# KirillHit/snn_for_object_detection

Measured on AMD Instinct MI355X. Metric: event-frames/sec (BxT) SODa-3M GEN1 304x240 fwd+bwd, higher is better.
Workload: dtype f32 (16-bit split products)

## Files before the change

include/snn_hip.h:

```cpp
#ifndef SNN_HIP_H
#define SNN_HIP_H

#include <stddef.h>
#include <stdint.h>

#ifdef __cplusplus
extern "C" {
#endif

#define SNN_ABI_VERSION 20

enum {
    SNN_NEURON_NONE = 0,
    SNN_NEURON_LIF = 1,
    SNN_NEURON_LI = 2,
    SNN_NEURON_LI_TANH = 3,
    SNN_NEURON_SLI = 4,
    SNN_NEURON_SYNAPSE = 5
};

enum { SNN_PREC_FP32 = 0, SNN_PREC_BF16X3 = 1, SNN_PREC_BF16X6 = 3, SNN_PREC_FP16X3 = 4, SNN_PREC_BF16X1 = 5,
       SNN_PREC_BF16S = 6 };

enum { SNN_SCAN_WIDE_ADDRESSING = 1,
// ... 66 lines not shown
                     int64_t N, int H, int W, int Cin, int Ho, int Wo, int Cout,
                     int KH, int KW, int stride, int pad, const float* addend, int64_t ld_addend,
                     const float* addend2, int64_t ld_addend2, int precision, void* stream);
int snn_conv2d_wgrad(const float* x, int64_t ldx, const float* dy, int64_t lddy, float* dw,
                     int64_t N, int H, int W, int Cin, int Ho, int Wo, int Cout,
                     int KH, int KW, int stride, int pad, int accumulate,
                     float* workspace, int splitk, int precision, void* stream);
int snn_conv2d_wgrad_splitk(int64_t N, int H, int W, int Cin, int Ho, int Wo, int Cout, int KH, int KW,
                            int stride, int pad, int precision);
int snn_conv2d_wgrad_kernel(int64_t N, int H, int W, int Cin, int Ho, int Wo, int Cout, int KH, int KW, int stride, int pad,
                            int precision);
int snn_conv2d_gather_plan(int mode, int64_t N, int H, int W, int Cin, int Ho, int Wo, int Cout, int KH, int KW, int stride,
                           int pad, int64_t ld_in, int64_t ld_out, int align_bits, int has_split_image, int has_addend,
                           int has_addend2, int frames_per_step, int precision, int phase, int* out);
int snn_conv2d_wgrad_plan(int64_t N, int H, int W, int Cin, int Ho, int Wo, int Cout, int KH, int KW, int stride, int pad,
                          int64_t ldx, int64_t lddy, int align_bits, int precision, int spikes, int num_cu, int* out);
int snn_conv1x1_spikes_supported(int64_t N, int H, int W, int Cin, int Cout, int64_t ld, int fwd_precision,
                                 int bwd_precision);
int snn_conv1x1_spikes_fwd(const float* vdec, int64_t ld, float v_th, const float* w, float* y, int64_t ldy, int64_t N, int H,
                           int W, int Cin, int Cout, void* stream);
int snn_conv1x1_spikes_wgrad(const float* vdec, int64_t ld, float v_th, const float* dy, int64_t lddy, float* dw, int64_t N,
                             int H, int W, int Cin, int Cout, int accumulate, float* workspace, int splitk, void* stream);

int snn_conv2d_spikes_supported(int64_t N, int H, int W, int Cin, int Ho, int Wo, int Cout, int KH, int KW, int stride,
                                int pad, int64_t ld, int fwd_precision, int bwd_precision);
int snn_conv2d_spikes_fwd(const float* vdec, int64_t ld, float v_th, const float* w, float* y, int64_t ldy, int64_t N, int H,
                          int W, int Cin, int Ho, int Wo, int Cout, int KH, int KW, int stride, int pad, double* bn_partial,
                          int frames_per_step, int* bn_layout, void* stream);
int snn_conv2d_spikes_wgrad(const float* vdec, int64_t ld, float v_th, const float* dy, int64_t lddy, float* dw, int64_t N,
                            int H, int W, int Cin, int Ho, int Wo, int Cout, int KH, int KW, int stride, int pad,
                            int accumulate, float* workspace, int splitk, void* stream);
int snn_conv3x3_halo_spikes(const float* vdec, int64_t ld, float v_th, const void* w_image, float* y, int64_t ldy, int64_t N,
                            int H, int W, int Cin, int Cout, double* bn_partial, int frames_per_step, int* bn_layout,
                            void* stream);

size_t snn_bn_stats_partial_size(int T, int64_t M, int C);
int snn_bn_stats(const float* y, int64_t ldy, int T, int64_t M, int C, double* partial, void* stream);
int snn_bn_stats_finalize(const double* partial, int chunks, int rows_per_chunk, int T, int64_t M, int C,
                          const float* gamma, const float* bias, float eps, float momentum,
                          float* running_mean, float* running_var, int use_running,
                          float* mean, float* invstd, float* alpha, float* beta, void* stream);

int snn_bn_stats_reduce(const double* partial, int chunks, int rows_per_chunk, int T, int64_t M, int C, double* sums,
                        void* stream);
int snn_bn_stats_from_sums(const double* sums, int T, int64_t M_total, int C,
                           const float* gamma, const float* bias, float eps, float momentum,
// ... 161 lines not shown
```

snn_for_object_detection_amd/_build.py:

```python

import hashlib
import json
import os
import shutil
import subprocess
import sys
from concurrent.futures import ThreadPoolExecutor

HERE = os.path.dirname(os.path.abspath(__file__))
CSRC = os.path.join(HERE, "csrc")
INCLUDE = os.path.join(os.path.dirname(HERE), "include")
SCRATCH = os.path.join(os.path.dirname(HERE), "build")
LIB_NAME = "libsnn_hip.so"
LIB_PATH = os.path.join(HERE, LIB_NAME)
STAMP_PATH = LIB_PATH + ".buildstamp"
SOURCES = ("elementwise.hip", "neuron.hip", "conv.hip", "wgrad_halo.hip", "conv_halo.hip", "detect.hip",
           "targets.hip", "metrics.hip")
HEADERS = (os.path.join(CSRC, "snn_common.h"), os.path.join(INCLUDE, "snn_hip.h"))
ARCH = "gfx950"
FLAGS = ["-O3", f"--offload-arch={ARCH}", "-fPIC", "-ffp-contract=off", "-std=c++17", "-Wall",
         "-Wno-unused-function", f"-I{INCLUDE}"]


def _hipcc() -> str:
    for cand in (os.environ.get("HIPCC"), shutil.which("hipcc"), "/opt/rocm/bin/hipcc"):
        if cand and os.path.exists(cand):
            return cand
    raise RuntimeError("hipcc not found: the HIP extension cannot be built")


def _sha(*chunks: bytes) -> str:
    h = hashlib.sha256()
    for c in chunks:
        h.update(c)
    return h.hexdigest()


def source_fingerprint() -> str:
    h = hashlib.sha256()
# ... 128 lines not shown
```

snn_for_object_detection_amd/_hip.py:

```python

import ctypes
import os
from ctypes import POINTER, Structure, c_char_p, c_double, c_float, c_int, c_int32, c_int64, c_size_t, c_void_p

_HERE = os.path.dirname(os.path.abspath(__file__))
LIB_PATH = os.environ.get("SNN_HIP_LIB") or os.path.join(_HERE, "libsnn_hip.so")

NEURON_NONE, NEURON_LIF, NEURON_LI, NEURON_LI_TANH, NEURON_SLI, NEURON_SYNAPSE = 0, 1, 2, 3, 4, 5
POOL_AVG, POOL_MAX, POOL_SUM = 0, 1, 2
ACT_RELU, ACT_SILU, ACT_TANH = 0, 1, 2
ABI_VERSION = 20
PREC_FP32, PREC_BF16X3, PREC_BF16X6, PREC_FP16X3, PREC_BF16X1, PREC_BF16S = 0, 1, 3, 4, 5, 6
SCAN_WIDE_ADDRESSING, SCAN_LAST_STEP_ONLY, SCAN_BF16_STORAGE, SCAN_SPIKES_FROM_VDEC, SCAN_SUMS_FROM_STATE = 1, 2, 4, 8, 16
SCAN_STATE_LOOKBACK = 32
SURR_SUPER, SURR_TRIANGLE, SURR_SIGMOID, SURR_ATAN = 0, 1, 2, 3


class NeuronParams(Structure):
    _fields_ = [("c_mem", c_float), ("c_syn", c_float), ("v_leak", c_float), ("v_th", c_float),
                ("v_reset", c_float), ("alpha", c_float), ("v_st", c_float), ("tau_sec", c_float),
                ("tau_dis", c_float), ("dt", c_float), ("sigma", c_float),
                ("surrogate", c_int), ("reset_detached", c_int)]


# ... 20 lines not shown
                                    _P, _I, _P]),
    "snn_conv3x3_s2_dgrad_supported": (c_int, [_L, _I, _I, _I, _I, _I, _I]),
    "snn_conv3x3_s2_dgrad_plan": (c_int, [_L, _I, _I, _I, _I, _I, _I, _P]),
    "snn_conv3x3_halo_plan": (c_int, [_L, _I, _I, _I, _I, _I, _P]),
    "snn_conv2d_wgrad_halo_plan": (c_int, [_L, _I, _I, _I, _I, _I, _I, _I, _I, _P]),
    "snn_conv_first_plan": (c_int, [_L, _I, _I, _I, _I, _I, _I, _I, _I, _I, _I, _P]),
    "snn_conv3x3_s2_dgrad": (c_int, [_P, _L, _P, _P, _L, _L, _I, _I, _I, _I, _I, _I, _P, _L, _P, _L, _I, _P]),
    "snn_conv3x3_halo_supported": (c_int, [_L, _I, _I, _I, _I]),
    "snn_conv3x3_halo_bn_chunks": (c_int64, [_I, _I, _I]),
    "snn_weight_frag_image_bytes": (c_size_t, [_I, _I]),
    "snn_weight_frag_image_batched": (c_int, [_P, _P, _P, _I, _I, _I, _I, _P]),
    "snn_conv3x3_halo": (c_int, [_P, _L, _P, _P, _L, _L, _I, _I, _I, _I, _P, _L, _P, _L, _P, _I, _P, _I, _P]),
    "snn_conv2d_dgrad": (c_int, [_P, _L, _P, _P, _P, _L, _L, _I, _I, _I, _I, _I, _I, _I, _I, _I, _I, _P, _L, _P, _L,
                                 _I, _P]),
    "snn_conv2d_wgrad": (c_int, [_P, _L, _P, _L, _P, _L, _I, _I, _I, _I, _I, _I, _I, _I, _I, _I, _I, _P, _I, _I,
                                 _P]),
    "snn_conv2d_wgrad_splitk": (c_int, [_L, _I, _I, _I, _I, _I, _I, _I, _I, _I, _I, _I]),
    "snn_conv2d_wgrad_kernel": (c_int, [_L, _I, _I, _I, _I, _I, _I, _I, _I, _I, _I, _I]),
    "snn_conv2d_gather_plan": (c_int, [_I, _L, _I, _I, _I, _I, _I, _I, _I, _I, _I, _I, _L, _L, _I, _I, _I, _I, _I, _I, _I, _P]),
    "snn_conv2d_wgrad_plan": (c_int, [_L, _I, _I, _I, _I, _I, _I, _I, _I, _I, _I, _L, _L, _I, _I, _I, _I, _P]),
    "snn_conv1x1_spikes_supported": (c_int, [_L, _I, _I, _I, _I, _L, _I, _I]),
    "snn_conv1x1_spikes_fwd": (c_int, [_P, _L, _F, _P, _P, _L, _L, _I, _I, _I, _I, _P]),
    "snn_conv1x1_spikes_wgrad": (c_int, [_P, _L, _F, _P, _L, _P, _L, _I, _I, _I, _I, _I, _P, _I, _P]),
    "snn_conv2d_spikes_supported": (c_int, [_L, _I, _I, _I, _I, _I, _I, _I, _I, _I, _I, _L, _I, _I]),
    "snn_conv2d_spikes_fwd": (c_int, [_P, _L, _F, _P, _P, _L, _L, _I, _I, _I, _I, _I, _I, _I, _I, _I, _I, _P, _I, _P, _P]),
    "snn_conv2d_spikes_wgrad": (c_int, [_P, _L, _F, _P, _L, _P, _L, _I, _I, _I, _I, _I, _I, _I, _I, _I, _I, _I, _P, _I, _P]),
    "snn_conv3x3_halo_spikes": (c_int, [_P, _L, _F, _P, _P, _L, _L, _I, _I, _I, _I, _P, _I, _P, _P]),
    "snn_bn_stats_partial_size": (c_size_t, [_I, _L, _I]),
    "snn_bn_stats": (c_int, [_P, _L, _I, _L, _I, _P, _P]),
    "snn_bn_stats_finalize": (c_int, [_P, _I, _I, _I, _L, _I, _P, _P, _F, _F, _P, _P, _I, _P, _P, _P, _P, _P]),
    "snn_bn_stats_reduce": (c_int, [_P, _I, _I, _I, _L, _I, _P, _P]),
    "snn_bn_stats_from_sums": (c_int, [_P, _I, _L, _I, _P, _P, _F, _F, _P, _P, _P, _P, _P, _P, _P, _P]),
    "snn_bn_bwd_reduce": (c_int, [_P, _I, _L, _I, _P, _P]),
    "snn_bn_bwd_coef": (c_int, [_P, _P, _P, _I, _L, _I, _P, _P, _P, _P, _P, _P, _P, _P, _I, _P]),
    "snn_affine_neuron_fwd": (c_int, [_I, _P, _L, _P, _P, _P, _P, _P, _L, _P, _L, _P, _P, _P, _I, _L, _I,
                                      POINTER(NeuronParams), _I, _P]),
    "snn_lif_ckpt_interval": (c_int, []),
    "snn_lif_fwd_ckpt": (c_int, [_P, _L, _P, _P, _P, _P, _P, _L, _P, _L, _P, _P, _P, _I, _L, _I,
                                 POINTER(NeuronParams), _P]),
    "snn_lif_bwd_ckpt": (c_int, [_P, _L, _P, _P, _L, _P, _P, _P, _P, _I, _P, _P, _P, _P, _I, _L, _I,
                                 POINTER(NeuronParams), _P]),
    "snn_affine_neuron_bwd_sums_size": (c_size_t, [_I, _L, _I]),
    "snn_affine_neuron_bwd": (c_int, [_I, _P, _L, _P, _P, _L, _P, _P, _P, _P, _I, _P, _P, _P, _P, _I, _L, _I,
                                      POINTER(NeuronParams), _I, _P]),
    "snn_bn_bwd_finalize": (c_int, [_P, _I, _L, _I, _P, _P, _P, _P, _P, _P, _P, _P, _I, _P]),
    "snn_bn_bwd_finalize_from_state": (c_int, [_P, _I, _L, _I, _P, _P, _P, _P, _P, _P, _L, _P, _P, _P, _P, _P, _I, _P]),
# ... 91 lines not shown
```

snn_for_object_detection_amd/csrc/conv.hip:

```cpp
#include <stdlib.h>
#include <type_traits>
#include "snn_common.h"

#if defined(SNN_STAMP) || defined(SNN_CLOCK)
__device__ unsigned long long g_stamps[2048 * 8];
__device__ unsigned long long g_stamps2[2048 * 4];
extern "C" int snn_debug_stamps(unsigned long long* out, int n) {
    return (int)hipMemcpyFromSymbol(out, HIP_SYMBOL(g_stamps), sizeof(unsigned long long) * n);
}
extern "C" int snn_debug_stamps2(unsigned long long* out, int n) {
    return (int)hipMemcpyFromSymbol(out, HIP_SYMBOL(g_stamps2), sizeof(unsigned long long) * n);
}
#endif
#ifdef SNN_STAMP
#define STAMP(i) do { unsigned long long t_ = __builtin_readcyclecounter(); st_acc[i] += t_ - st_last; st_last = t_; } while (0)
#else
#define STAMP(i) do {} while (0)
#endif

namespace {

constexpr int kThreads = 256;
constexpr int BM = 128;
constexpr int BK = 32;
// ... 2070 lines not shown
        hipLaunchKernelGGL(k_wgrad_reduce4, dim3((unsigned)r.blocks, 1), dim3(kThreads), 0, st, workspace, n,
                           r.groups, r.groups, (int64_t)r.per * n, dw, 0, accumulate);
        SNN_CHECK_LAUNCH("snn_conv2d_wgrad_reduce");
        return 0;
    }
    if (r.kind == kReduce4OnePass) {
        hipLaunchKernelGGL(k_wgrad_reduce4, dim3((unsigned)r.blocks, 1), dim3(kThreads), 0, st, workspace, n, splitk,
                           splitk, n, dw, 0, accumulate);
        SNN_CHECK_LAUNCH("snn_conv2d_wgrad_reduce");
        return 0;
    }
    const bool launched = dispatch(
        [&](auto KG) {
            hipLaunchKernelGGL((k_wgrad_reduce<KG()>), dim3((unsigned)r.blocks), dim3(kThreads), 0, st, workspace, dw, n, splitk,
                               accumulate);
            return true;
        },
        OneOf<1, 4, 16, 64>{r.kg});
    SNN_REQUIRE(launched, "snn_conv2d_wgrad_reduce: no kernel for %d thread groups", r.kg);
    SNN_CHECK_LAUNCH("snn_conv2d_wgrad_reduce");
    return 0;
}

namespace {
static FirstPlan first_layer_wgrad_plan(unsigned align, int64_t ldx, int64_t lddy, int64_t N, int H, int W, int Cin, int Ho,
                                        int Wo, int Cout, int KH, int KW, int stride, int pad, bool dy_bf16, int num_cu) {
    if (Cin != 2 || KH != 3 || KW != 3) return FirstPlan{};
    FirstPlan p = first_layer_plan(N, H, W, Ho, Wo, Cout, stride, pad, 0, true, num_cu);
    if (!(ldx % 2 == 0 && (align & kAlignIn8) && lddy % 4 == 0 && (align & (dy_bf16 ? kAlignDy8 : kAlignDy16)) &&
          (int64_t)W * ldx < 0x7fffffffLL))
        p.ok = 0;
    return p;
}
static unsigned wgrad_align_bits(const void* x, const void* dy) {
    return (aligned(16, {x}) ? kAlignIn16 : 0u) | (aligned(8, {x}) ? kAlignIn8 : 0u) | (aligned(16, {dy}) ? kAlignDy16 : 0u) |
           (aligned(8, {dy}) ? kAlignDy8 : 0u);
}
static FirstPlan first_layer_wgrad_plan(const float* x, int64_t ldx, const float* dy, int64_t lddy, int64_t N, int H, int W,
                                        int Cin, int Ho, int Wo, int Cout, int KH, int KW, int stride, int pad) {
    return first_layer_wgrad_plan(wgrad_align_bits(x, dy), ldx, lddy, N, H, W, Cin, Ho, Wo, Cout, KH, KW, stride, pad, false, 0);
}

enum WgradKernel { kWgradPipe = 0, kWgradVec = 1, kWgradScalar = 2, kWgradHalo = 3, kWgradFirst = 4 };
enum WgradRefusal { kWgradOk = 0, kWgradHaloSplitk, kWgradNotPipeSB, kWgradNotPipeXSP, kWgradGridTooLarge };
struct WgradPlan {
    int ok, why;
// ... 280 lines not shown
```

snn_for_object_detection_amd/csrc/snn_common.h:

```cpp
#pragma once
#include <hip/hip_runtime.h>
#include <stdint.h>
#include <stdio.h>
#include <initializer_list>
#include <type_traits>
#include "../../include/snn_hip.h"

void snn_set_error(const char* fmt, ...);

#define SNN_REQUIRE(cond, ...)            \
    do {                                  \
        if (!(cond)) {                    \
            snn_set_error(__VA_ARGS__);   \
            return 1;                     \
        }                                 \
    } while (0)

#define SNN_CHECK_LAUNCH(name)                                                   \
    do {                                                                         \
        hipError_t e_ = hipGetLastError();                                       \
        if (e_ != hipSuccess) {                                                  \
            snn_set_error("%s: launch failed: %s", name, hipGetErrorString(e_)); \
            return 2;                                                            \
        }                                                                        \
// ... 39 lines not shown

#ifdef SNN_TUNING
#include <stdlib.h>
static inline const char* snn_tuning_env(const char* name) { return getenv(name); }
#else
static inline const char* snn_tuning_env(const char*) { return nullptr; }
#endif

struct SnnWgradHaloPlan {
    int ok;
    int R, CW, npr, npc, nks;
    int HR, HC, HWD, HWD2;
    int wco, wk;
    int tiles_co, tiles_ci, splits, pps, patches;
    int slabs;
};
SnnWgradHaloPlan snn_wgrad_halo_plan(int64_t N, int H, int W, int Cin, int Ho, int Wo, int Cout, int KH, int KW,
                                     int stride, int pad, int num_cu = 0);
int snn_wgrad_halo_launch(const SnnWgradHaloPlan& p, const float* x, int64_t ldx, const float* dy, int64_t lddy,
                          float* workspace, int64_t N, int H, int W, int Cin, int Ho, int Wo, int Cout, int stride,
                          int nprod , bool bf16_storage ,
                          hipStream_t st, float x_th = 0.0f);

typedef float f32x4 __attribute__((ext_vector_type(4)));

__host__ __device__ inline int64_t snn_bn_partial_index(int64_t t, int64_t chunk, int64_t c, int64_t chunks, int64_t C) {
    return ((t * C + c) * chunks + chunk) * 2;
}
typedef float f32x16 __attribute__((ext_vector_type(16)));

#ifdef __HIPCC__
typedef unsigned snn_u32x2 __attribute__((ext_vector_type(2)));
typedef __bf16 snn_bf16x2 __attribute__((ext_vector_type(2)));
typedef float snn_f32x2 __attribute__((ext_vector_type(2)));
__device__ __forceinline__ f32x4 snn_unpack_bf16x4(snn_u32x2 r) {
    f32x4 v;
    v[0] = __builtin_bit_cast(float, r[0] << 16);
    v[1] = __builtin_bit_cast(float, r[0] & 0xffff0000u);
    v[2] = __builtin_bit_cast(float, r[1] << 16);
    v[3] = __builtin_bit_cast(float, r[1] & 0xffff0000u);
    return v;
}
__device__ __forceinline__ snn_u32x2 snn_pack_bf16x4(f32x4 v) {
    const snn_bf16x2 a = __builtin_convertvector(snn_f32x2{v[0], v[1]}, snn_bf16x2);
    const snn_bf16x2 b = __builtin_convertvector(snn_f32x2{v[2], v[3]}, snn_bf16x2);
    return snn_u32x2{__builtin_bit_cast(unsigned, a), __builtin_bit_cast(unsigned, b)};
// ... 37 lines not shown
```

snn_for_object_detection_amd/functional.py:

```python

import collections
import ctypes
import os
from typing import List, NamedTuple, Optional, Sequence, Tuple

import torch
from torch.autograd import Function

from . import _hip
from ._hip import NeuronParams

_F32 = torch.float32
DEFAULT_DT = 0.001


SURROGATES = {"super": _hip.SURR_SUPER, "triangle": _hip.SURR_TRIANGLE, "sigmoid": _hip.SURR_SIGMOID,
              "atan": _hip.SURR_ATAN}


def _surrogate_code(surrogate: str) -> int:
    if surrogate not in SURROGATES:
        raise ValueError(f"unknown surrogate {surrogate!r}: one of {sorted(SURROGATES)}")
    return SURROGATES[surrogate]

# ... 499 lines not shown

    def deposit(self, key, g: torch.Tensor, exclusive: bool = False) -> None:
        if self.result is None and g is not None:
            self.deposits[key] = g
            if exclusive:
                self.exclusive.add(key)

    def set_result(self, dx: torch.Tensor) -> None:
        self.result = dx


def _acc_of(x):
    return getattr(x, "_snn_acc", None)


def _same_tensor(a: torch.Tensor, b: torch.Tensor) -> bool:
    return (a.data_ptr() == b.data_ptr() and tuple(a.shape) == tuple(b.shape) and a.stride() == b.stride())


def _slot_of(param) -> Optional[GradSlot]:
    return getattr(param, "_snn_grad_slot", None) if param is not None else None


def _dgrad_accumulate(acc, gy, ldg, wt, x, geom, st, prec, wt_split=None, wt_image=None):
    T, B, Cin, H, W, Cout, KH, KW, Ho, Wo, stride, pad = geom
    dx, dx_shape = None, (T, B, Cin, H, W)
    addend, ld_add, addend2, ld_add2 = None, 0, None, 0
    outer_fused = None
    if acc is not None and acc[0].result is None and acc[0].deposits:
        key, other = next(iter(acc[0].deposits.items()))
        other = _raw_to_cl(other)
        if tuple(other.shape) == dx_shape:
            addend, ld_add = other.data_ptr(), cl_stride(other)
            acc[0].fused[key] = acc[0].deposits.pop(key)
    if (acc is not None and acc[0].result is None and not acc[0].deposits and acc[0].outer is not None
            and FUSE_OUTER_ADDEND):
        o_acc, o_key = acc[0].outer
        if o_acc.result is None and len(o_acc.deposits) == 1 and o_key not in o_acc.deposits:
            key2, other2 = next(iter(o_acc.deposits.items()))
            other2 = _raw_to_cl(other2)
            if tuple(other2.shape) == dx_shape:
                addend2, ld_add2 = other2.data_ptr(), cl_stride(other2)
                outer_fused = (o_acc, o_key, key2)
                if (o_acc.grad_in_slot and key2 in o_acc.exclusive and other2.dtype == x.dtype and ld_add2 % 4 == 0
                        and USE_SIBLING_FUSION):
                    dx = _alias(other2, other2.storage_offset(), T, B, Cin, H, W, ld_add2)
    chained = False
    if (acc is not None and acc[0].result is not None and addend is None and acc[1] not in acc[0].fused
            and tuple(acc[0].result.shape) == dx_shape):
        prev = acc[0].result
        addend, ld_add = prev.data_ptr(), cl_stride(prev)
        chained = True
    if dx is None:
        dx = _new_cl((T, B), Cin, H, W, x)
    if (prec in _HALO_BWD_PRECS and _halo_operand_ok(gy.data_ptr(), ldg, prec == _hip.PREC_BF16S) and USE_HALO_CONV
            and (KH, KW, stride, pad) == (3, 3, 2, 1)
            and _hip.query("snn_conv3x3_s2_dgrad_supported", T * B, H, W, Cin, Ho, Wo, Cout)):
        if wt_image is None:
            wt_image = _frag_image(wt, Cin, Cout, 1, _hip.PREC_BF16X3)
        _hip.call("snn_conv3x3_s2_dgrad", gy.data_ptr(), ldg, wt_image.data_ptr(), dx.data_ptr(), cl_stride(dx), T * B, H, W, Cin, Ho,
                  Wo, Cout, addend, ld_add, addend2, ld_add2, prec, st)
    elif (prec in _HALO_BWD_PRECS and _halo_operand_ok(gy.data_ptr(), ldg, prec == _hip.PREC_BF16S)
            and _halo_ok(T * B, H, W, Cout, Cin, KH, KW, stride, pad)):
        if wt_image is None:
            wt_image = _frag_image(wt, Cin, Cout, 1, _hip.PREC_BF16X3)
        _hip.call("snn_conv3x3_halo", gy.data_ptr(), ldg, wt_image.data_ptr(), dx.data_ptr(), cl_stride(dx), T * B, H, W, Cout,
                  Cin, addend, ld_add, addend2, ld_add2, None, 0, None, prec, st)
    else:
        _hip.call("snn_conv2d_dgrad", gy.data_ptr(), ldg, wt.data_ptr(), wt_split, dx.data_ptr(), cl_stride(dx), T * B, H, W,
                  Cin, Ho, Wo, Cout, KH, KW, stride, pad, addend, ld_add, addend2, ld_add2, prec, st)
    if acc is not None and (acc[0].result is None or chained):
        if chained and acc[0].outer is not None and acc[0].outer[0].result is acc[0].result:
            acc[0].outer[0].set_result(dx)
            acc[0].outer[0].fused[acc[0].outer[1]] = dx
        acc[0].set_result(dx)
        acc[0].fused[acc[1]] = dx
    if outer_fused is not None:
        o_acc, o_key, key2 = outer_fused
        o_acc.fused[key2] = o_acc.deposits.pop(key2)
        o_acc.fused[o_key] = dx
        o_acc.set_result(dx)
    return dx


USE_HALO_CONV = not os.environ.get("SNN_NO_HALO_CONV")
_HALO_BWD_PRECS = (_hip.PREC_BF16X3, _hip.PREC_BF16S)


def _halo_ok(N: int, H: int, W: int, Cin: int, Cout: int, KH: int, KW: int, stride: int, pad: int) -> bool:
    return (USE_HALO_CONV and KH == 3 and KW == 3 and stride == 1 and pad == 1
            and bool(_hip.query("snn_conv3x3_halo_supported", N, H, W, Cin, Cout)))


# ... 146 lines not shown
        if pend is not None:
            fused = (not ctx.needs_input_grad[0] and ctx.needs_input_grad[1] and ctx.slot is not None
                     and pend.gx.dtype == _F32 and pend.dims == (T, B, Cout, Ho, Wo) and cl_stride(pend.y) % 4 == 0
                     and _hip.query("snn_conv2d_wgrad_bn_supported", T * B, H, W, Cin, Ho, Wo, Cout, KH, KW, stride, pad))
            if fused:
                splitk = _hip.query("snn_conv2d_wgrad_splitk", T * B, H, W, Cin, Ho, Wo, Cout, KH, KW, stride, pad, ctx.prec)
                with _WgradLaunch(x.device, True, splitk, Cout, KH * KW * Cin,
                                   hold=(x, pend.gx, pend.y, pend.coef)) as (stream, ws, _):
                    _hip.call("snn_conv2d_wgrad_bn", x.data_ptr(), ldx, pend.gx.data_ptr(), Cout, pend.y.data_ptr(),
                              cl_stride(pend.y), pend.coef.data_ptr(), T, B, ctx.slot.buf.data_ptr(), T * B, H, W, Cin, Ho,
                              Wo, Cout, KH, KW, stride, pad, ctx.slot.claim(), ws.data_ptr(), splitk, stream)
                return None, None, None, None, None, None, None, None, None, None
            _apply_pending(pend)
        if ctx.needs_input_grad[0]:
            wt = _kept_view(ctx.weight, "_snn_wt")
            wt16 = wt_img = None
            if wt is not None:
                wt_img = _kept_view(ctx.weight, "_snn_wtfrag")
                if ctx.prec == _hip.PREC_BF16X3 and USE_PRESPLIT_WEIGHTS and USE_PRESPLIT_DGRAD:
                    wt16 = _ptr(_kept_view(ctx.weight, "_snn_wt16"))
            else:
                wt = torch.empty((Cin, KH, KW, Cout), device=x.device, dtype=_F32)
                _hip.call("snn_weight_transpose", w_ohwi.data_ptr(), wt.data_ptr(), Cout, KH, KW, Cin, st)
            dx = _dgrad_accumulate(ctx.acc, gy, ldg, wt, x, ctx.geom, st, ctx.prec, wt_split=wt16, wt_image=wt_img)
        if ctx.needs_input_grad[1]:
            splitk = _hip.query("snn_conv2d_wgrad_splitk", T * B, H, W, Cin, Ho, Wo, Cout, KH, KW, stride, pad, ctx.prec)
            xw, ldxw, x_th = _spikes_wgrad_operand(x, ldx, ctx.x_th, gy, ldg)
            slot = ctx.slot
            with _WgradLaunch(x.device, slot is not None, splitk, Cout, KH * KW * Cin,
                              hold=(x, xw, gy)) as (stream, ws, _):
                if slot is not None:
                    dst, accumulate = slot.buf, slot.claim()
                else:
                    dst, accumulate = torch.empty((Cout, KH, KW, Cin), device=x.device, dtype=_F32), 0
                if x_th is not None:
                    _hip.call("snn_conv2d_spikes_wgrad", xw.data_ptr(), ldxw, x_th, gy.data_ptr(), ldg, dst.data_ptr(),
                              T * B, H, W, Cin, Ho, Wo, Cout, KH, KW, stride, pad, accumulate, ws.data_ptr(), splitk,
                              stream)
                else:
                    _hip.call("snn_conv2d_wgrad", xw.data_ptr(), ldxw, gy.data_ptr(), ldg, dst.data_ptr(), T * B, H, W,
                              Cin, Ho, Wo, Cout, KH, KW, stride, pad, accumulate, ws.data_ptr(), splitk, ctx.prec,
                              stream)
            if slot is None:
                dw = dst.permute(0, 3, 1, 2)
        return dx, dw, None, None, None, None, None, None, None, None


# ... 126 lines not shown
        else:
            _hip.call("snn_conv2d_fwd", x.data_ptr(), cl_stride(x), wc.data_ptr(), None, y.data_ptr(), cl_stride(y), T * B,
                      H, W, Cin, H, W, Ct, 1, 1, 1, 0, None, 0, None, 0, None, fwd_prec, _stream())
        ctx.prec = bwd_prec
        ctx.x_th = x_th
        ctx.save_for_backward(x, w1m, *w2ms)
        ctx.wct = wct
        ctx.geom = (T, B, Cin, H, W, Ct, 1, 1, H, W, 1, 0)
        ctx.widths, ctx.c1 = widths, C1
        ctx.slot1, ctx.slots2 = slot1, slots2
        ctx.acc = acc
        return y

    @staticmethod
    def backward(ctx, gy):
        x, w1m, *w2ms = ctx.saved_tensors
        T, B, Cin, H, W, Ct = ctx.geom[:6]
        C1, widths = ctx.c1, ctx.widths
        composed = w1m is not None
        gy = _raw_to_cl(gy)
        ldg, ldx = cl_stride(gy), cl_stride(x)
        dx = dw1 = None
        dw2s = [None] * len(widths)
        if ctx.needs_input_grad[0]:
            dx = _dgrad_accumulate(ctx.acc, gy, ldg, ctx.wct, x, ctx.geom, _stream(), ctx.prec)
        if any(ctx.needs_input_grad[8:]) or (composed and ctx.needs_input_grad[1]):
            slot1, slots2 = ctx.slot1, ctx.slots2
            slotted = all(s_ is not None for s_ in slots2) and (slot1 is not None or not composed)
            splitk = _hip.query("snn_conv2d_wgrad_splitk", T * B, H, W, Cin, H, W, Ct, 1, 1, 1, 0, ctx.prec)
            xw, ldxw, x_th = _spikes_wgrad_operand(x, ldx, ctx.x_th, gy, ldg)
            with _WgradLaunch(x.device, slotted, splitk, Ct, Cin, hold=(x, xw, gy), with_g=True) as (stream, ws, G):
                if x_th is not None:
                    _hip.call("snn_conv1x1_spikes_wgrad", xw.data_ptr(), ldxw, x_th, gy.data_ptr(), ldg, G.data_ptr(),
                              T * B, H, W, Cin, Ct, 0, ws.data_ptr(), splitk, stream)
                else:
                    _hip.call("snn_conv2d_wgrad", xw.data_ptr(), ldxw, gy.data_ptr(), ldg, G.data_ptr(), T * B, H, W,
                              Cin, H, W, Ct, 1, 1, 1, 0, 0, ws.data_ptr(), splitk, ctx.prec, stream)
                g1 = None
                if composed:
                    g1 = slot1.buf.view(C1, Cin) if slotted else torch.empty((C1, Cin), device=x.device, dtype=_F32)
                    acc1 = slot1.claim() if slotted else 0
                row = 0
                for b, (w2m, c) in enumerate(zip(w2ms, widths)):
                    Gb = G[row:row + c]
                    row += c
                    if slotted:
                        g2, acc2 = slots2[b].buf.view(c, C1), slots2[b].claim()
                    else:
                        g2, acc2 = torch.empty((c, C1), device=x.device, dtype=_F32), 0
                    if composed:
                        _small_gemm(Gb, False, w1m, True, g2, acc2)
                        _small_gemm(w2m, True, Gb, False, g1, acc1)
                        acc1 = 1
                    elif acc2:
                        g2.add_(Gb)
# ... 1010 lines not shown
```

snn_for_object_detection_amd/profiler.py:

```python

from collections import defaultdict
from typing import Dict

import torch


WGRAD_LABELS = ("k_conv_wgrad_pipe", "k_conv_wgrad_halo", "k_conv_first<wgrad>")


def _wgrad_label(n, h, w, cin, ho, wo, cout, kh, kw, stride, pad, prec) -> str:
    from . import _hip
    return WGRAD_LABELS[int(_hip.query("snn_conv2d_wgrad_kernel", n, h, w, cin, ho, wo, cout, kh, kw, stride, pad, prec))]


def _conv_label(name: str, a) -> str:
    if name == "snn_conv2d_wgrad":
        return _wgrad_label(a[5], a[6], a[7], a[8], a[9], a[10], a[11], a[12], a[13], a[14], a[15], a[19])
    dgrad = name == "snn_conv2d_dgrad"
    cin, cout = a[8], a[11]
    oc, ic = (cin, cout) if dgrad else (cout, cin)
    if not dgrad and cin == 2 and a[12] == 3 and a[13] == 3 and cout % 4 == 0 and (cout // 4) & (cout // 4 - 1) == 0 \
            and cout <= 256 and a[16] is None:
        return "k_conv_first<2, 3, false>"
    if oc <= 32:
# ... 5 lines not shown
    return f"k_conv_gather<{tile}, {'true' if dgrad else 'false'}, {'true' if ic % 4 == 0 else 'false'}>"


PREC_BF16S, SCAN_BF16_STORAGE = 6, 4


def work_of(name: str, a):
    if name in ("snn_conv2d_fwd", "snn_conv2d_dgrad"):
        a = tuple(a[:3]) + tuple(a[4:])
        n, h, w, cin, ho, wo, cout, kh, kw = a[5], a[6], a[7], a[8], a[9], a[10], a[11], a[12], a[13]
        sb = a[21 if name == "snn_conv2d_fwd" else 20] == PREC_BF16S
        es = 2.0 if sb else 4.0
        es_in = 4.0 if (cin == 2 and name == "snn_conv2d_fwd") else es
        flops = 2.0 * n * ho * wo * cout * kh * kw * cin
        byts = es_in * n * h * w * cin + es * n * ho * wo * cout + 4.0 * cout * kh * kw * cin
        return _conv_label(name, a) + (", bf16s" if sb else ""), flops, byts
    if name == "snn_conv2d_wgrad":
        n, h, w, cin, ho, wo, cout, kh, kw = a[5], a[6], a[7], a[8], a[9], a[10], a[11], a[12], a[13]
        sb = a[19] == PREC_BF16S
        es = 2.0 if sb else 4.0
        flops = 2.0 * n * ho * wo * cout * kh * kw * cin
        byts = (4.0 if cin == 2 else es) * n * h * w * cin + es * n * ho * wo * cout + 4.0 * cout * kh * kw * cin
        return _conv_label(name, a) + (", bf16s" if sb else ""), flops, byts
    if name in ("snn_conv1x1_spikes_fwd", "snn_conv1x1_spikes_wgrad"):
        fwd = name.endswith("_fwd")
        n, h, w, cin, cout = (a[6], a[7], a[8], a[9], a[10])
        flops = 2.0 * n * h * w * cout * cin
        byts = 4.0 * (n * h * w * cin + n * h * w * cout + cout * cin)
        if not fwd:
            return WGRAD_LABELS[0], flops, byts
        tile = "32, 4, 1" if cout <= 32 else ("64, 2, 2" if cout <= 64 else "128, 2, 2")
        return f"k_conv_gather<{tile}, false, true>", flops, byts
    if name in ("snn_conv2d_spikes_fwd", "snn_conv2d_spikes_wgrad"):
        fwd = name.endswith("_fwd")
        n, h, w, cin, ho, wo, cout, kh, kw, stride, pad = a[6:17]
        flops = 2.0 * n * ho * wo * cout * kh * kw * cin
        byts = 4.0 * (n * h * w * cin + n * ho * wo * cout + cout * kh * kw * cin)
        if not fwd:
            return _wgrad_label(n, h, w, cin, ho, wo, cout, kh, kw, stride, pad, 1) + ", spikes", flops, byts
        tile = "32, 4, 1" if cout <= 32 else ("64, 2, 2" if cout <= 64 else "128, 2, 2")
        return f"k_conv_gather<{tile}, false, true>", flops, byts
    if name == "snn_conv3x3_halo_spikes":
        n, h, w, cin, cout = a[6], a[7], a[8], a[9], a[10]
        flops = 2.0 * n * h * w * cout * 9 * cin
        byts = 4.0 * (n * h * w * cin + n * h * w * cout) + 4.0 * cout * 9 * cin
        return f"k_conv_halo3<{128 if cout % 128 == 0 else (64 if cout % 64 == 0 else 32)}, fwd, spikes>", flops, byts
# ... 104 lines not shown
```

Before: 7218.

## Fuse 1x1 conv dgrad and wgrad into one kernel sharing the dy tile

Adds a HIP kernel that computes both the input gradient and per-block weight-gradient partials of a 1x1 convolution in a single pass over dy, staging dy and x tiles in LDS as split bf16 hi/lo pairs and using MFMA. The partial slabs are then reduced by the existing split-k reduce. The aim is to stop reading dy twice (separate dgrad and wgrad kernels) and to drop the separate spike-operand preparation. In exchange it adds register and LDS pressure, a workspace allocation per call and an extra reduce launch.

```diff
diff --git a/include/snn_hip.h b/include/snn_hip.h
--- a/include/snn_hip.h
+++ b/include/snn_hip.h
@@ -112,6 +112,13 @@
 int snn_conv1x1_spikes_wgrad(const float* vdec, int64_t ld, float v_th, const float* dy, int64_t lddy, float* dw, int64_t N,
                              int H, int W, int Cin, int Cout, int accumulate, float* workspace, int splitk, void* stream);
 
+int snn_conv1x1_bwd_supported(const void* dy, int64_t lddy, const void* x, int64_t ldx, int64_t lddx, int64_t N, int H, int W,
+                              int Cin, int Cout, int precision, int64_t min_pixels);
+int snn_conv1x1_bwd(const float* dy, int64_t lddy, const float* x, int64_t ldx, int spikes, float x_th, const float* wt,
+                    float* dx, int64_t lddx, const float* addend, int64_t ld_add, const float* addend2, int64_t ld_add2,
+                    float* workspace, int slabs, int64_t N, int H, int W, int Cin, int Cout, int precision, void* stream);
+int snn_conv1x1_bwd_reduce(float* workspace, int slabs, float* dw, int Cin, int Cout, int accumulate, void* stream);
+
 int snn_conv2d_spikes_supported(int64_t N, int H, int W, int Cin, int Ho, int Wo, int Cout, int KH, int KW, int stride,
                                 int pad, int64_t ld, int fwd_precision, int bwd_precision);
 int snn_conv2d_spikes_fwd(const float* vdec, int64_t ld, float v_th, const float* w, float* y, int64_t ldy, int64_t N, int H,
diff --git a/snn_for_object_detection_amd/_build.py b/snn_for_object_detection_amd/_build.py
--- a/snn_for_object_detection_amd/_build.py
+++ b/snn_for_object_detection_amd/_build.py
@@ -14,7 +14,7 @@
 LIB_NAME = "libsnn_hip.so"
 LIB_PATH = os.path.join(HERE, LIB_NAME)
 STAMP_PATH = LIB_PATH + ".buildstamp"
-SOURCES = ("elementwise.hip", "neuron.hip", "conv.hip", "wgrad_halo.hip", "conv_halo.hip", "detect.hip",
+SOURCES = ("elementwise.hip", "neuron.hip", "conv.hip", "conv1x1_bwd.hip", "wgrad_halo.hip", "conv_halo.hip", "detect.hip",
            "targets.hip", "metrics.hip")
 HEADERS = (os.path.join(CSRC, "snn_common.h"), os.path.join(INCLUDE, "snn_hip.h"))
 ARCH = "gfx950"
diff --git a/snn_for_object_detection_amd/_hip.py b/snn_for_object_detection_amd/_hip.py
--- a/snn_for_object_detection_amd/_hip.py
+++ b/snn_for_object_detection_amd/_hip.py
@@ -66,6 +66,9 @@
     "snn_conv1x1_spikes_supported": (c_int, [_L, _I, _I, _I, _I, _L, _I, _I]),
     "snn_conv1x1_spikes_fwd": (c_int, [_P, _L, _F, _P, _P, _L, _L, _I, _I, _I, _I, _P]),
     "snn_conv1x1_spikes_wgrad": (c_int, [_P, _L, _F, _P, _L, _P, _L, _I, _I, _I, _I, _I, _P, _I, _P]),
+    "snn_conv1x1_bwd_supported": (c_int, [_P, _L, _P, _L, _L, _L, _I, _I, _I, _I, _I, _L]),
+    "snn_conv1x1_bwd": (c_int, [_P, _L, _P, _L, _I, _F, _P, _P, _L, _P, _L, _P, _L, _P, _I, _L, _I, _I, _I, _I, _I, _P]),
+    "snn_conv1x1_bwd_reduce": (c_int, [_P, _I, _P, _I, _I, _I, _P]),
     "snn_conv2d_spikes_supported": (c_int, [_L, _I, _I, _I, _I, _I, _I, _I, _I, _I, _I, _L, _I, _I]),
     "snn_conv2d_spikes_fwd": (c_int, [_P, _L, _F, _P, _P, _L, _L, _I, _I, _I, _I, _I, _I, _I, _I, _I, _I, _P, _I, _P, _P]),
     "snn_conv2d_spikes_wgrad": (c_int, [_P, _L, _F, _P, _L, _P, _L, _I, _I, _I, _I, _I, _I, _I, _I, _I, _I, _I, _P, _I, _P]),
diff --git a/snn_for_object_detection_amd/csrc/conv.hip b/snn_for_object_detection_amd/csrc/conv.hip
--- a/snn_for_object_detection_amd/csrc/conv.hip
+++ b/snn_for_object_detection_amd/csrc/conv.hip
@@ -2116,6 +2116,10 @@
     return 0;
 }
 
+int snn_wgrad_reduce_slabs(float* workspace, float* dw, int64_t n, int splitk, int accumulate, hipStream_t st) {
+    return wgrad_reduce_slabs(workspace, dw, n, splitk, accumulate, st);
+}
+
 namespace {
 static FirstPlan first_layer_wgrad_plan(unsigned align, int64_t ldx, int64_t lddy, int64_t N, int H, int W, int Cin, int Ho,
                                         int Wo, int Cout, int KH, int KW, int stride, int pad, bool dy_bf16, int num_cu) {
diff --git a/snn_for_object_detection_amd/csrc/conv1x1_bwd.hip b/snn_for_object_detection_amd/csrc/conv1x1_bwd.hip
--- /dev/null
+++ b/snn_for_object_detection_amd/csrc/conv1x1_bwd.hip
@@ -0,0 +1,297 @@
+#include "snn_common.h"
+
+namespace {
+
+constexpr int kThreads = 256;
+constexpr int PB = 32;
+constexpr int LDT = PB + 8;
+constexpr int kBlocksPerCu = 2;
+
+typedef __bf16 bf16x8 __attribute__((ext_vector_type(8)));
+typedef __bf16 bf16x4 __attribute__((ext_vector_type(4)));
+typedef __bf16 bf16x2 __attribute__((ext_vector_type(2)));
+typedef float f32x2 __attribute__((ext_vector_type(2)));
+
+struct Bwd1x1Geom {
+    int64_t M;
+    int64_t lddy, ldx, lddx, ld_add, ld_add2;
+    int pix_per_block;
+    float x_th;
+};
+
+__device__ __forceinline__ void split2(float a, float b, __bf16& ha, __bf16& hb, __bf16& la, __bf16& lb) {
+    f32x2 v = {a, b};
+    bf16x2 p = __builtin_convertvector(v, bf16x2);
+    const unsigned bits = __builtin_bit_cast(unsigned, p);
+    ha = p[0];
+    hb = p[1];
+    v[0] -= __builtin_bit_cast(float, bits << 16);
+    v[1] -= __builtin_bit_cast(float, bits & 0xffff0000u);
+    p = __builtin_convertvector(v, bf16x2);
+    la = p[0];
+    lb = p[1];
+}
+
+template <int CI, int CO, bool XSP>
+__global__ __launch_bounds__(kThreads, kBlocksPerCu) void k_conv1x1_dgrad_wgrad(
+    const float* __restrict__ dy, const float* __restrict__ x, const float* __restrict__ wt, float* dx,
+    const float* addend, const float* addend2, float* __restrict__ ws, Bwd1x1Geom g) {
+    static_assert(CI % 32 == 0 && CI <= 128 && CO % 32 == 0 && CO <= 128, "channel tiles");
+    constexpr int LDR = CO + 8;
+    constexpr int NT = CI / 32;
+    constexpr int MTC = CO / 32;
+    constexpr int DWT = MTC * NT;
+    constexpr int TPW = (DWT + 3) / 4;
+    constexpr int KS = CO / 16;
+    constexpr int NITEM = 2 * (CO + CI);
+    constexpr int NQI = (NITEM + kThreads - 1) / kThreads;
+    __shared__ __attribute__((aligned(16))) __bf16 Rh[PB * LDR];
+    __shared__ __attribute__((aligned(16))) __bf16 Rl[PB * LDR];
+    __shared__ __attribute__((aligned(16))) __bf16 Dh[CO * LDT];
+    __shared__ __attribute__((aligned(16))) __bf16 Dl[CO * LDT];
+    __shared__ __attribute__((aligned(16))) __bf16 Xh[CI * LDT];
+    __shared__ __attribute__((aligned(16))) __bf16 Xl[XSP ? 8 : CI * LDT];
+
+    const int tid = threadIdx.x;
+    const int lane_id = tid & 63, wave = tid >> 6;
+    const int r = lane_id & 31, h = lane_id >> 5;
+
+    const int64_t p_lo = (int64_t)blockIdx.x * g.pix_per_block;
+    int n = 0;
+    if (p_lo < g.M) n = (int)(g.M - p_lo < (int64_t)g.pix_per_block ? g.M - p_lo : (int64_t)g.pix_per_block);
+
+    __amdgpu_buffer_rsrc_t rs_d, rs_x;
+    {
+        const int64_t dbytes = n > 0 ? ((int64_t)(n - 1) * g.lddy + CO) * 4 : 0;
+        const int64_t xbytes = n > 0 ? ((int64_t)(n - 1) * g.ldx + CI) * 4 : 0;
+        rs_d = __builtin_amdgcn_make_buffer_rsrc(const_cast<float*>(dy + p_lo * g.lddy), 0, (int)dbytes, 0x00020000);
+        rs_x = __builtin_amdgcn_make_buffer_rsrc(const_cast<float*>(x + p_lo * g.ldx), 0, (int)xbytes, 0x00020000);
+    }
+
+    int it_off[NQI];
+    int it_row[NQI];
+    int it_ch[NQI];
+#pragma unroll
+    for (int q = 0; q < NQI; ++q) {
+        const int it = tid + kThreads * q;
+        const bool is_d = it < 2 * CO;
+        const int j = is_d ? it : it - 2 * CO;
+        it_row[q] = ((j >> 2) & 7) * 4;
+        it_ch[q] = ((j & 3) + 4 * (j >> 5)) * 4;
+        const int ld = (int)(is_d ? g.lddy : g.ldx);
+        it_off[q] = it < NITEM ? (it_row[q] * ld + it_ch[q]) * 4 : -1;
+    }
+    f32x4 rv[NQI][4];
+    auto load_stage = [&](int s0) {
+#pragma unroll
+        for (int q = 0; q < NQI; ++q) {
+            const bool is_d = tid + kThreads * q < 2 * CO;
+            const int ld4 = (int)(is_d ? g.lddy : g.ldx) * 4;
+#pragma unroll
+            for (int e = 0; e < 4; ++e) {
+                const int voff = it_off[q] < 0 ? -1 : it_off[q] + (s0 + e) * ld4;
+                rv[q][e] = __builtin_bit_cast(f32x4, is_d ? __builtin_amdgcn_raw_buffer_load_b128(rs_d, voff, 0, 0)
+                                                          : __builtin_amdgcn_raw_buffer_load_b128(rs_x, voff, 0, 0));
+            }
+        }
+    };
+    auto write_stage = [&]() {
+#pragma unroll
+        for (int q = 0; q < NQI; ++q) {
+            const int it = tid + kThreads * q;
+            if (it >= NITEM) continue;
+            const bool is_d = it < 2 * CO;
+            const int row = it_row[q], ch = it_ch[q];
+            if (is_d || !XSP) {
+                __bf16 hi[4][4], lo[4][4];
+#pragma unroll
+                for (int e = 0; e < 4; ++e)
+#pragma unroll
+                    for (int c = 0; c < 4; c += 2)
+                        split2(rv[q][e][c], rv[q][e][c + 1], hi[e][c], hi[e][c + 1], lo[e][c], lo[e][c + 1]);
+                __bf16* Th = is_d ? Dh : Xh;
+                __bf16* Tl = is_d ? Dl : Xl;
+#pragma unroll
+                for (int c = 0; c < 4; ++c) {
+                    *reinterpret_cast<bf16x4*>(&Th[(ch + c) * LDT + row]) = bf16x4{hi[0][c], hi[1][c], hi[2][c], hi[3][c]};
+                    *reinterpret_cast<bf16x4*>(&Tl[(ch + c) * LDT + row]) = bf16x4{lo[0][c], lo[1][c], lo[2][c], lo[3][c]};
+                }
+                if (is_d) {
+#pragma unroll
+                    for (int e = 0; e < 4; ++e) {
+                        *reinterpret_cast<bf16x4*>(&Rh[(row + e) * LDR + ch]) = bf16x4{hi[e][0], hi[e][1], hi[e][2], hi[e][3]};
+                        *reinterpret_cast<bf16x4*>(&Rl[(row + e) * LDR + ch]) = bf16x4{lo[e][0], lo[e][1], lo[e][2], lo[e][3]};
+                    }
+                }
+            } else {
+#pragma unroll
+                for (int c = 0; c < 4; ++c) {
+                    snn_u32x2 o;
+#pragma unroll
+                    for (int e = 0; e < 4; e += 2)
+                        o[e >> 1] = (rv[q][e][c] > g.x_th ? 0x3F80u : 0u) | (rv[q][e + 1][c] > g.x_th ? 0x3F800000u : 0u);
+                    *reinterpret_cast<snn_u32x2*>(&Xh[(ch + c) * LDT + row]) = o;
+                }
+            }
+        }
+    };
+
+    bf16x8 wh[KS], wl[KS];
+    if (wave < NT) {
+        const float* wrow = wt + (int64_t)(wave * 32 + r) * CO + 8 * h;
+#pragma unroll
+        for (int ks = 0; ks < KS; ++ks)
+#pragma unroll
+            for (int i = 0; i < 8; i += 2) {
+                __bf16 ha, hb, la, lb;
+                split2(wrow[ks * 16 + i], wrow[ks * 16 + i + 1], ha, hb, la, lb);
+                wh[ks][i] = ha; wh[ks][i + 1] = hb;
+                wl[ks][i] = la; wl[ks][i + 1] = lb;
+            }
+    }
+
+    f32x16 dwacc[TPW];
+#pragma unroll
+    for (int i = 0; i < TPW; ++i)
+#pragma unroll
+        for (int e = 0; e < 16; ++e) dwacc[i][e] = 0.f;
+
+    if (n > 0) load_stage(0);
+#pragma unroll 1
+    for (int s0 = 0; s0 < n; s0 += PB) {
+        write_stage();
+        __syncthreads();
+        load_stage(s0 + PB);
+
+        if (wave < NT) {
+            const int ci = wave * 32 + r;
+            float add[16];
+#pragma unroll
+            for (int e = 0; e < 16; ++e) {
+                const int p = s0 + (e & 3) + 8 * (e >> 2) + 4 * h;
+                float a = 0.f;
+                if (p < n) {
+                    if (addend) a = __builtin_nontemporal_load(addend + (p_lo + p) * g.ld_add + ci);
+                    if (addend2) a += __builtin_nontemporal_load(addend2 + (p_lo + p) * g.ld_add2 + ci);
+                }
+                add[e] = a;
+            }
+            f32x16 acc;
+#pragma unroll
+            for (int e = 0; e < 16; ++e) acc[e] = 0.f;
+#pragma unroll
+            for (int ks = 0; ks < KS; ++ks) {
+                const int off = r * LDR + ks * 16 + 8 * h;
+                const bf16x8 ah = *reinterpret_cast<const bf16x8*>(&Rh[off]);
+                const bf16x8 al = *reinterpret_cast<const bf16x8*>(&Rl[off]);
+                acc = __builtin_amdgcn_mfma_f32_32x32x16_bf16(al, wh[ks], acc, 0, 0, 0);
+                acc = __builtin_amdgcn_mfma_f32_32x32x16_bf16(ah, wl[ks], acc, 0, 0, 0);
+                acc = __builtin_amdgcn_mfma_f32_32x32x16_bf16(ah, wh[ks], acc, 0, 0, 0);
+            }
+#pragma unroll
+            for (int e = 0; e < 16; ++e) {
+                const int p = s0 + (e & 3) + 8 * (e >> 2) + 4 * h;
+                if (p < n) dx[(p_lo + p) * g.lddx + ci] = acc[e] + add[e];
+            }
+        }
+#pragma unroll
+        for (int i = 0; i < TPW; ++i) {
+            const int t = wave + 4 * i;
+            if (t < DWT) {
+                const int mt = t % MTC, nt = t / MTC;
+#pragma unroll
+                for (int ks = 0; ks < PB / 16; ++ks) {
+                    const int offd = (mt * 32 + r) * LDT + ks * 16 + 8 * h;
+                    const int offx = (nt * 32 + r) * LDT + ks * 16 + 8 * h;
+                    const bf16x8 ah = *reinterpret_cast<const bf16x8*>(&Dh[offd]);
+                    const bf16x8 al = *reinterpret_cast<const bf16x8*>(&Dl[offd]);
+                    const bf16x8 bh = *reinterpret_cast<const bf16x8*>(&Xh[offx]);
+                    dwacc[i] = __builtin_amdgcn_mfma_f32_32x32x16_bf16(al, bh, dwacc[i], 0, 0, 0);
+                    if constexpr (!XSP) {
+                        const bf16x8 bl = *reinterpret_cast<const bf16x8*>(&Xl[offx]);
+                        dwacc[i] = __builtin_amdgcn_mfma_f32_32x32x16_bf16(ah, bl, dwacc[i], 0, 0, 0);
+                    }
+                    dwacc[i] = __builtin_amdgcn_mfma_f32_32x32x16_bf16(ah, bh, dwacc[i], 0, 0, 0);
+                }
+            }
+        }
+        __syncthreads();
+    }
+
+    float* slab = ws + (int64_t)blockIdx.x * (CO * CI);
+#pragma unroll
+    for (int i = 0; i < TPW; ++i) {
+        const int t = wave + 4 * i;
+        if (t < DWT) {
+            const int mt = t % MTC, nt = t / MTC;
+#pragma unroll
+            for (int e = 0; e < 16; ++e) {
+                const int co = mt * 32 + (e & 3) + 8 * (e >> 2) + 4 * h;
+                slab[co * CI + nt * 32 + r] = dwacc[i][e];
+            }
+        }
+    }
+}
+
+struct Bwd1x1Plan {
+    int blocks;
+    int pix_per_block;
+};
+
+static Bwd1x1Plan bwd1x1_plan(const void* dy, int64_t lddy, const void* x, int64_t ldx, int64_t lddx, int64_t N, int H, int W,
+                              int Cin, int Cout, int precision, int64_t min_pixels, int num_cu) {
+    Bwd1x1Plan p = {0, 0};
+    const int64_t M = N * (int64_t)H * W;
+    auto chan_ok = [](int c) { return c == 32 || c == 64 || c == 128; };
+    if (precision != SNN_PREC_BF16X3 || M <= 0 || M >= 0x7fffffffLL || !chan_ok(Cin) || !chan_ok(Cout)) return p;
+    if (!multiples(4, {lddy, ldx, lddx}) || lddy < Cout || ldx < Cin || lddx < Cin || !aligned(16, {dy, x})) return p;
+    const int64_t stages = snn_ceil_div(M, PB);
+    int64_t blocks = (int64_t)(num_cu > 0 ? num_cu : snn_num_cu()) * kBlocksPerCu;
+    if (blocks > stages) blocks = stages;
+    const int64_t ppb = snn_ceil_div(stages, blocks) * PB;
+    if ((ppb + 2 * PB) * (lddy > ldx ? lddy : ldx) * 4 >= 0x7fffffffLL) return p;
+    if (M < (min_pixels < 0 ? 2 * blocks * Cin : min_pixels)) return p;
+    p.blocks = (int)blocks;
+    p.pix_per_block = (int)ppb;
+    return p;
+}
+
+}
+
+extern "C" int snn_conv1x1_bwd_supported(const void* dy, int64_t lddy, const void* x, int64_t ldx, int64_t lddx, int64_t N,
+                                         int H, int W, int Cin, int Cout, int precision, int64_t min_pixels) {
+    return bwd1x1_plan(dy, lddy, x, ldx, lddx, N, H, W, Cin, Cout, precision, min_pixels, 0).blocks;
+}
+
+extern "C" int snn_conv1x1_bwd(const float* dy, int64_t lddy, const float* x, int64_t ldx, int spikes, float x_th,
+                               const float* wt, float* dx, int64_t lddx, const float* addend, int64_t ld_add,
+                               const float* addend2, int64_t ld_add2, float* workspace, int slabs, int64_t N, int H, int W,
+                               int Cin, int Cout, int precision, void* stream) {
+    SNN_REQUIRE(dy && x && wt && dx && workspace, "snn_conv1x1_bwd: null pointer");
+    const Bwd1x1Plan p = bwd1x1_plan(dy, lddy, x, ldx, lddx, N, H, W, Cin, Cout, precision, 0, 0);
+    SNN_REQUIRE(p.blocks > 0, "snn_conv1x1_bwd: shape, strides or alignment not covered (ask snn_conv1x1_bwd_supported): "
+                "N=%lld %dx%d %d->%d lddy=%lld ldx=%lld lddx=%lld precision=%d", (long long)N, H, W, Cin, Cout, (long long)lddy,
+                (long long)ldx, (long long)lddx, precision);
+    SNN_REQUIRE(slabs == p.blocks, "snn_conv1x1_bwd: workspace of %d slabs, the plan writes %d", slabs, p.blocks);
+    SNN_REQUIRE((!addend || ld_add >= Cin) && (!addend2 || ld_add2 >= Cin), "snn_conv1x1_bwd: addend pixel stride below Cin");
+    Bwd1x1Geom g;
+    g.M = N * (int64_t)H * W;
+    g.lddy = lddy; g.ldx = ldx; g.lddx = lddx; g.ld_add = ld_add; g.ld_add2 = ld_add2;
+    g.pix_per_block = p.pix_per_block;
+    g.x_th = x_th;
+    const bool launched = dispatch(
+        [&](auto CI, auto CO, auto XSP) {
+            hipLaunchKernelGGL((k_conv1x1_dgrad_wgrad<CI(), CO(), XSP()>), dim3((unsigned)p.blocks), dim3(kThreads), 0,
+                               (hipStream_t)stream, dy, x, wt, dx, addend, addend2, workspace, g);
+            return true;
+        },
+        OneOf<32, 64, 128>{Cin}, OneOf<32, 64, 128>{Cout}, Flag{spikes != 0});
+    SNN_REQUIRE(launched, "snn_conv1x1_bwd: no kernel for %d -> %d channels", Cin, Cout);
+    SNN_CHECK_LAUNCH("snn_conv1x1_bwd");
+    return 0;
+}
+
+extern "C" int snn_conv1x1_bwd_reduce(float* workspace, int slabs, float* dw, int Cin, int Cout, int accumulate, void* stream) {
+    SNN_REQUIRE(workspace && dw && slabs > 0, "snn_conv1x1_bwd_reduce: null pointer or no slabs");
+    return snn_wgrad_reduce_slabs(workspace, dw, (int64_t)Cin * Cout, slabs, accumulate, (hipStream_t)stream);
+}
diff --git a/snn_for_object_detection_amd/csrc/snn_common.h b/snn_for_object_detection_amd/csrc/snn_common.h
--- a/snn_for_object_detection_amd/csrc/snn_common.h
+++ b/snn_for_object_detection_amd/csrc/snn_common.h
@@ -85,6 +85,8 @@
                           int nprod , bool bf16_storage ,
                           hipStream_t st, float x_th = 0.0f);
 
+int snn_wgrad_reduce_slabs(float* workspace, float* dw, int64_t n, int splitk, int accumulate, hipStream_t st);
+
 typedef float f32x4 __attribute__((ext_vector_type(4)));
 
 __host__ __device__ inline int64_t snn_bn_partial_index(int64_t t, int64_t chunk, int64_t c, int64_t chunks, int64_t C) {
diff --git a/snn_for_object_detection_amd/functional.py b/snn_for_object_detection_amd/functional.py
--- a/snn_for_object_detection_amd/functional.py
+++ b/snn_for_object_detection_amd/functional.py
@@ -545,7 +545,31 @@
     return getattr(param, "_snn_grad_slot", None) if param is not None else None
 
 
-def _dgrad_accumulate(acc, gy, ldg, wt, x, geom, st, prec, wt_split=None, wt_image=None):
+USE_FUSED_1X1_BWD = not os.environ.get("SNN_NO_FUSED_1X1_BWD")
+FUSED_1X1_MIN_PIXELS = -1
+
+
+class FusedWgrad:
+
+    __slots__ = ("x_th", "ws")
+
+    def __init__(self, x_th: Optional[float]):
+        self.x_th, self.ws = x_th, None
+
+
+def _fused_wgrad_request(geom, gy, x, prec, x_th) -> Optional[FusedWgrad]:
+    T, B, Cin, H, W, Cout, KH, KW, Ho, Wo, stride, pad = geom
+    if (USE_FUSED_1X1_BWD and (KH, KW, stride, pad) == (1, 1, 1, 0) and prec == _hip.PREC_BF16X3 and gy.dtype == _F32
+            and x.dtype == _F32):
+        return FusedWgrad(x_th)
+    return None
+
+
+def _fused_wgrad_reduce(fw: FusedWgrad, dst: torch.Tensor, Cin: int, Cout: int, accumulate: int, stream: int) -> None:
+    _hip.call("snn_conv1x1_bwd_reduce", fw.ws.data_ptr(), fw.ws.shape[0], dst.data_ptr(), Cin, Cout, accumulate, stream)
+
+
+def _dgrad_accumulate(acc, gy, ldg, wt, x, geom, st, prec, wt_split=None, wt_image=None, fused_wgrad=None):
     T, B, Cin, H, W, Cout, KH, KW, Ho, Wo, stride, pad = geom
     dx, dx_shape = None, (T, B, Cin, H, W)
     addend, ld_add, addend2, ld_add2 = None, 0, None, 0
@@ -590,8 +614,19 @@
         _hip.call("snn_conv3x3_halo", gy.data_ptr(), ldg, wt_image.data_ptr(), dx.data_ptr(), cl_stride(dx), T * B, H, W, Cout,
                   Cin, addend, ld_add, addend2, ld_add2, None, 0, None, prec, st)
     else:
-        _hip.call("snn_conv2d_dgrad", gy.data_ptr(), ldg, wt.data_ptr(), wt_split, dx.data_ptr(), cl_stride(dx), T * B, H, W,
-                  Cin, Ho, Wo, Cout, KH, KW, stride, pad, addend, ld_add, addend2, ld_add2, prec, st)
+        slabs = 0
+        if fused_wgrad is not None:
+            slabs = _hip.query("snn_conv1x1_bwd_supported", gy.data_ptr(), ldg, x.data_ptr(), cl_stride(x), cl_stride(dx),
+                               T * B, H, W, Cin, Cout, prec, FUSED_1X1_MIN_PIXELS)
+        if slabs:
+            fw = fused_wgrad
+            fw.ws = torch.empty((slabs, Cout * Cin), device=x.device, dtype=_F32)
+            _hip.call("snn_conv1x1_bwd", gy.data_ptr(), ldg, x.data_ptr(), cl_stride(x), int(fw.x_th is not None),
+                      float(fw.x_th or 0.0), wt.data_ptr(), dx.data_ptr(), cl_stride(dx), addend, ld_add, addend2, ld_add2,
+                      fw.ws.data_ptr(), slabs, T * B, H, W, Cin, Cout, prec, st)
+        else:
+            _hip.call("snn_conv2d_dgrad", gy.data_ptr(), ldg, wt.data_ptr(), wt_split, dx.data_ptr(), cl_stride(dx), T * B, H,
+                      W, Cin, Ho, Wo, Cout, KH, KW, stride, pad, addend, ld_add, addend2, ld_add2, prec, st)
     if acc is not None and (acc[0].result is None or chained):
         if chained and acc[0].outer is not None and acc[0].outer[0].result is acc[0].result:
             acc[0].outer[0].set_result(dx)
@@ -784,7 +819,15 @@
             else:
                 wt = torch.empty((Cin, KH, KW, Cout), device=x.device, dtype=_F32)
                 _hip.call("snn_weight_transpose", w_ohwi.data_ptr(), wt.data_ptr(), Cout, KH, KW, Cin, st)
-            dx = _dgrad_accumulate(ctx.acc, gy, ldg, wt, x, ctx.geom, st, ctx.prec, wt_split=wt16, wt_image=wt_img)
+            fw = None
+            if ctx.needs_input_grad[1] and ctx.slot is not None:
+                fw = _fused_wgrad_request(ctx.geom, gy, x, ctx.prec, ctx.x_th)
+            dx = _dgrad_accumulate(ctx.acc, gy, ldg, wt, x, ctx.geom, st, ctx.prec, wt_split=wt16, wt_image=wt_img,
+                                   fused_wgrad=fw)
+            if fw is not None and fw.ws is not None:
+                with _WgradLaunch(x.device, True, 0, Cout, Cin, hold=(fw.ws,)) as (stream, _, _):
+                    _fused_wgrad_reduce(fw, ctx.slot.buf, Cin, Cout, ctx.slot.claim(), stream)
+                return dx, None, None, None, None, None, None, None, None, None
         if ctx.needs_input_grad[1]:
             splitk = _hip.query("snn_conv2d_wgrad_splitk", T * B, H, W, Cin, Ho, Wo, Cout, KH, KW, stride, pad, ctx.prec)
             xw, ldxw, x_th = _spikes_wgrad_operand(x, ldx, ctx.x_th, gy, ldg)
@@ -957,15 +1000,26 @@
         ldg, ldx = cl_stride(gy), cl_stride(x)
         dx = dw1 = None
         dw2s = [None] * len(widths)
+        want_w = any(ctx.needs_input_grad[8:]) or (composed and ctx.needs_input_grad[1])
+        fw = None
         if ctx.needs_input_grad[0]:
-            dx = _dgrad_accumulate(ctx.acc, gy, ldg, ctx.wct, x, ctx.geom, _stream(), ctx.prec)
-        if any(ctx.needs_input_grad[8:]) or (composed and ctx.needs_input_grad[1]):
+            if want_w:
+                fw = _fused_wgrad_request(ctx.geom, gy, x, ctx.prec, ctx.x_th)
+            dx = _dgrad_accumulate(ctx.acc, gy, ldg, ctx.wct, x, ctx.geom, _stream(), ctx.prec, fused_wgrad=fw)
+        fused = fw is not None and fw.ws is not None
+        if want_w:
             slot1, slots2 = ctx.slot1, ctx.slots2
             slotted = all(s_ is not None for s_ in slots2) and (slot1 is not None or not composed)
-            splitk = _hip.query("snn_conv2d_wgrad_splitk", T * B, H, W, Cin, H, W, Ct, 1, 1, 1, 0, ctx.prec)
-            xw, ldxw, x_th = _spikes_wgrad_operand(x, ldx, ctx.x_th, gy, ldg)
-            with _WgradLaunch(x.device, slotted, splitk, Ct, Cin, hold=(x, xw, gy), with_g=True) as (stream, ws, G):
-                if x_th is not None:
+            if fused:
+                splitk, (xw, ldxw, x_th), hold = 0, (x, ldx, None), (fw.ws,)
+            else:
+                splitk = _hip.query("snn_conv2d_wgrad_splitk", T * B, H, W, Cin, H, W, Ct, 1, 1, 1, 0, ctx.prec)
+                xw, ldxw, x_th = _spikes_wgrad_operand(x, ldx, ctx.x_th, gy, ldg)
+                hold = (x, xw, gy)
+            with _WgradLaunch(x.device, slotted, splitk, Ct, Cin, hold=hold, with_g=True) as (stream, ws, G):
+                if fused:
+                    _fused_wgrad_reduce(fw, G, Cin, Ct, 0, stream)
+                elif x_th is not None:
                     _hip.call("snn_conv1x1_spikes_wgrad", xw.data_ptr(), ldxw, x_th, gy.data_ptr(), ldg, G.data_ptr(),
                               T * B, H, W, Cin, Ct, 0, ws.data_ptr(), splitk, stream)
                 else:
diff --git a/snn_for_object_detection_amd/profiler.py b/snn_for_object_detection_amd/profiler.py
--- a/snn_for_object_detection_amd/profiler.py
+++ b/snn_for_object_detection_amd/profiler.py
@@ -51,6 +51,13 @@
         flops = 2.0 * n * ho * wo * cout * kh * kw * cin
         byts = (4.0 if cin == 2 else es) * n * h * w * cin + es * n * ho * wo * cout + 4.0 * cout * kh * kw * cin
         return _conv_label(name, a) + (", bf16s" if sb else ""), flops, byts
+    if name == "snn_conv1x1_bwd":
+        n, h, w, cin, cout, slabs = a[15], a[16], a[17], a[18], a[19], a[14]
+        flops = 4.0 * n * h * w * cout * cin
+        byts = 4.0 * n * h * w * (cout + (2 + (a[9] is not None) + (a[11] is not None)) * cin) + 4.0 * (slabs + 1) * cout * cin
+        return f"k_conv1x1_dgrad_wgrad<{cin}, {cout}, {'true' if a[4] else 'false'}>", flops, byts
+    if name == "snn_conv1x1_bwd_reduce":
+        return "k_wgrad_reduce_once", 0.0, 4.0 * (a[1] + 1) * a[3] * a[4]
     if name in ("snn_conv1x1_spikes_fwd", "snn_conv1x1_spikes_wgrad"):
         fwd = name.endswith("_fwd")
         n, h, w, cin, cout = (a[6], a[7], a[8], a[9], a[10])
```

Result: no change. 7242, median of 6 (+0.3%).
